# deepspeedai/DeepSpeed

Measured on AMD Instinct MI355X. Metric: tokens/sec Llama-3-8B ZeRO-3, higher is better.
Workload: dtype bf16; 1 GPU; model=llama3-8b, global_batch=8, seq_len=4096, parallelism=zero3_dp1, grad_accum=2

## Files before the change

deepspeed_amd/ops/csrc/attention_bwd.hip:

```cpp
#include <torch/extension.h>

#include "common.h"

using bf16x8_t = __attribute__((ext_vector_type(8))) short;
using f32x4_t = __attribute__((ext_vector_type(4))) float;
using u32x4_t = __attribute__((ext_vector_type(4))) unsigned int;
using u32x2_t = __attribute__((ext_vector_type(2))) unsigned int;

#define MFMA_BF16_16x16x32 __builtin_amdgcn_mfma_f32_16x16x32_bf16

namespace bwd {

constexpr int BR = 128;
constexpr int WR = 32;
constexpr int KTW1 = 1;
constexpr int TS = 32;
constexpr int PT = 64;

DEV_INLINE unsigned int cvtpk2(float lo, float hi) {
  unsigned short a = __builtin_bit_cast(unsigned short, (__bf16)lo);
  unsigned short b = __builtin_bit_cast(unsigned short, (__bf16)hi);
  return (unsigned int)a | ((unsigned int)b << 16);
}

template <int DH>
__launch_bounds__(256)
__global__ void bwd_preprocess(
    const short* __restrict__ q, const short* __restrict__ k,
    const short* __restrict__ dout, const short* __restrict__ out,
    const float* __restrict__ lse,
    short* __restrict__ qT, short* __restrict__ doT, short* __restrict__ kT,
    float* __restrict__ drowP, float* __restrict__ lseP,
    int B, int S, int Sp, int Hq, int Hk) {
  constexpr int PPR = DH / 8;
  __shared__ unsigned int t[PT][DH / 2 + 1];

  const int z = blockIdx.z;
  const int H = (z == 2) ? Hk : Hq;
  const int bh = blockIdx.y;
  if (bh >= B * H) return;
  const int b = bh / H;
  const int h = bh % H;
  const int s0 = blockIdx.x * PT;
  const short* src = (z == 0) ? q : (z == 1) ? dout : k;
  short* dst = (z == 0) ? qT : (z == 1) ? doT : kT;

  for (int i = threadIdx.x; i < PT * PPR; i += 256) {
    const int row = i / PPR;
    const int c = i % PPR;
    const int s = s0 + row;
    const long long off = (((long long)b * S + s) * H + h) * DH + c * 8;
    u32x4_t x = {0u, 0u, 0u, 0u};
    if (s < S) x = *reinterpret_cast<const u32x4_t*>(src + off);
#pragma unroll
    for (int w = 0; w < 4; ++w) t[row][c * 4 + w] = x[w];
    if (z == 1) {
      u32x4_t o = {0u, 0u, 0u, 0u};
      if (s < S) o = *reinterpret_cast<const u32x4_t*>(out + off);
      float acc = 0.f;
#pragma unroll
      for (int w = 0; w < 4; ++w)
        acc += bf2f((short)(x[w] & 0xffff)) * bf2f((short)(o[w] & 0xffff)) +
               bf2f((short)(x[w] >> 16)) * bf2f((short)(o[w] >> 16));
#pragma unroll
      for (int m = PPR / 2; m > 0; m >>= 1) acc += __shfl_xor(acc, m, WAVE);
      if (c == 0) drowP[((long long)b * Hq + h) * Sp + s] = acc;
    } else if (z == 0 && c == 0) {
      float l = 0.f;
      if (s < S) {
        l = lse[((long long)b * Hq + h) * S + s];
        if (l == -INFINITY) l = INFINITY;
      }
      lseP[((long long)b * Hq + h) * Sp + s] = l;
    }
  }
  __syncthreads();
  for (int i = threadIdx.x; i < DH * (PT / 8); i += 256) {
    const int d = i / (PT / 8);
    const int pc = i % (PT / 8);
    const int sh = (d & 1) * 16;
    unsigned int e[8];
#pragma unroll
    for (int j = 0; j < 8; ++j) e[j] = (t[pc * 8 + j][d >> 1] >> sh) & 0xffffu;
    u32x4_t y = {e[0] | (e[1] << 16), e[2] | (e[3] << 16),
                 e[4] | (e[5] << 16), e[6] | (e[7] << 16)};
    *reinterpret_cast<u32x4_t*>(dst + (((long long)b * H + h) * DH + d) * Sp +
                                s0 + pc * 8) = y;
  }
}

template <int DH>
DEV_INLINE int rmswz(int row, int byte_off) {
  return row * (DH * 2) + (byte_off ^ ((row & 7) << 4));
}

DEV_INLINE void lds_dma16(const short* src, char* lds_wave_base) {
  __builtin_amdgcn_global_load_lds(
      reinterpret_cast<const unsigned int*>(src),
      reinterpret_cast<unsigned int*>(lds_wave_base), 16, 0, 0);
}

template <int DH>
DEV_INLINE void issue_rm(const short* base, long long rs, int r0, int S,
                         char* img, int sseg, int lane) {
  const int linear = sseg * 1024 + lane * 16;
  const int row = linear / (DH * 2);
  const int colbyte = linear % (DH * 2);
  const int src_col = colbyte ^ ((row & 7) << 4);
  const int grow = r0 + row;
  const int srow = grow < S ? grow : S - 1;
  lds_dma16(base + (long long)srow * rs + (src_col >> 1), img + sseg * 1024);
}

template <int DH>
DEV_INLINE void issue_tr(const short* baseT, int Sp, int c0, char* img,
                         int sseg, int lane) {
  const int linear = sseg * 1024 + lane * 16;
  const int d = linear >> 6;
  const int g = ((linear >> 4) & 3) ^ ((d >> 2) & 3);
  lds_dma16(baseT + (long long)d * Sp + c0 + g * 8, img + sseg * 1024);
}

template <int DH>
DEV_INLINE bf16x8_t read_rm(const char* img, int row, int ks, int l4) {
  return *reinterpret_cast<const bf16x8_t*>(
      img + rmswz<DH>(row, (l4 * 8 + 32 * ks) * 2));
}

DEV_INLINE bf16x8_t read_tr(const char* img, int d, int l4) {
  const int sw = (d >> 2) & 3;
  const char* rowp = img + d * 64 + (l4 & 1) * 8;
  u32x2_t lo = *reinterpret_cast<const u32x2_t*>(rowp + (((l4 >> 1) ^ sw) << 4));
  u32x2_t hi =
      *reinterpret_cast<const u32x2_t*>(rowp + (((2 + (l4 >> 1)) ^ sw) << 4));
  u32x4_t w = {lo[0], lo[1], hi[0], hi[1]};
  return __builtin_bit_cast(bf16x8_t, w);
}

DEV_INLINE bf16x8_t pack_pair(const f32x4_t& a, const f32x4_t& b) {
  u32x4_t w = {cvtpk2(a[0], a[1]), cvtpk2(a[2], a[3]), cvtpk2(b[0], b[1]),
               cvtpk2(b[2], b[3])};
  return __builtin_bit_cast(bf16x8_t, w);
}

DEV_INLINE void store4(short* p, const f32x4_t& a) {
  u32x2_t w = {cvtpk2(a[0], a[1]), cvtpk2(a[2], a[3])};
  *reinterpret_cast<u32x2_t*>(p) = w;
}

template <int NDT, int STRIDE>
DEV_INLINE void unrotate_row(f32x4_t* acc ,
                             const float* __restrict__ cr,
                             const float* __restrict__ sr) {
#pragma unroll
  for (int dt = 0; dt < NDT / 2; ++dt) {
    const f32x4_t c = *reinterpret_cast<const f32x4_t*>(cr + 16 * dt);
    const f32x4_t sn = *reinterpret_cast<const f32x4_t*>(sr + 16 * dt);
    const f32x4_t d1 = acc[dt * STRIDE];
    const f32x4_t d2 = acc[(dt + NDT / 2) * STRIDE];
    acc[dt * STRIDE] = d1 * c + d2 * sn;
    acc[(dt + NDT / 2) * STRIDE] = d2 * c - d1 * sn;
  }
}

template <int DH, int KTW, bool ROPE>
__launch_bounds__(512 / KTW, 1)
__global__ void flash_bwd_dkv_kernel(
    const short* __restrict__ q,
    const short* __restrict__ k,
    const short* __restrict__ v,
    const short* __restrict__ dout,
    const short* __restrict__ qT,
    const short* __restrict__ doT,
    const float* __restrict__ lseP,
    const float* __restrict__ drowP,
    const float* __restrict__ kvmask,
    short* __restrict__ dk,
    short* __restrict__ dv,
    const float* __restrict__ rope_cos,
    const float* __restrict__ rope_sin,
    int B, int S, int Sp, int Hq, int Hk, float scale, int causal) {
  constexpr int NKS = DH / 32;
  constexpr int NDT = DH / 16;
  constexpr int IMG = TS * DH * 2;
  constexpr int SPI = DH / 16;
  constexpr int NW = 8 / KTW;
  constexpr int WRK = 16 * KTW;
  constexpr int LD_OFF = 4 * IMG;
  constexpr int BUF = LD_OFF + 256;
  __shared__ __attribute__((aligned(16))) char smem[2 * BUF];

  const int lane = threadIdx.x & 63;
  const int wave = threadIdx.x >> 6;
  const int l15 = lane & 15;
  const int l4 = lane >> 4;

  const int bh = blockIdx.y;
  const int b = bh / Hk;
  const int hk = bh % Hk;
  const int G = Hq / Hk;
  const int kv_base = blockIdx.x * BR;
  const int wk = kv_base + wave * WRK;

  const long long qrs = (long long)Hq * DH;
  const long long kvrs = (long long)Hk * DH;
  const short* kp = k + ((long long)b * S) * kvrs + hk * DH;
  const short* vp = v + ((long long)b * S) * kvrs + hk * DH;

  bf16x8_t kfrag[KTW][NKS], vfrag[KTW][NKS];
  float maskv[KTW];
#pragma unroll
  for (int kt = 0; kt < KTW; ++kt) {
    const int krow = wk + 16 * kt + l15;
    const int srow = krow < S ? krow : S - 1;
    const short* ks = kp + (long long)srow * kvrs;
    const short* vs = vp + (long long)srow * kvrs;
#pragma unroll
    for (int ks_i = 0; ks_i < NKS; ++ks_i) {
      kfrag[kt][ks_i] =
          *reinterpret_cast<const bf16x8_t*>(ks + ks_i * 32 + l4 * 8);
      vfrag[kt][ks_i] =
          *reinterpret_cast<const bf16x8_t*>(vs + ks_i * 32 + l4 * 8);
    }
    maskv[kt] = (kvmask && krow < S) ? kvmask[(long long)b * S + krow] : 0.f;
  }

  f32x4_t dk_acc[NDT][KTW], dv_acc[NDT][KTW];
#pragma unroll
  for (int dt = 0; dt < NDT; ++dt)
#pragma unroll
    for (int kt = 0; kt < KTW; ++kt) {
      dk_acc[dt][kt] = f32x4_t{0.f, 0.f, 0.f, 0.f};
      dv_acc[dt][kt] = f32x4_t{0.f, 0.f, 0.f, 0.f};
    }

  const int q_start = causal ? kv_base : 0;
  const int nq = (S - q_start + TS - 1) / TS;
  const int total = G * nq;

  auto issue = [&](int g, int qb, int bufi) {
    const int h = hk * G + g;
    char* buf = smem + bufi * BUF;
    const short* qp = q + ((long long)b * S) * qrs + h * DH;
    const short* dop = dout + ((long long)b * S) * qrs + h * DH;
    const long long toff = ((long long)b * Hq + h) * DH * Sp;
    const long long roff = ((long long)b * Hq + h) * Sp;
#pragma unroll
    for (int sseg = wave; sseg < SPI; sseg += NW) {
      issue_rm<DH>(qp, qrs, qb, S, buf, sseg, lane);
      issue_rm<DH>(dop, qrs, qb, S, buf + IMG, sseg, lane);
      issue_tr<DH>(qT + toff, Sp, qb, buf + 2 * IMG, sseg, lane);
      issue_tr<DH>(doT + toff, Sp, qb, buf + 3 * IMG, sseg, lane);
    }
    if (wave == 0) {
      const float* s = (lane < 32 ? lseP : drowP) + roff + qb + (lane & 31);
      __builtin_amdgcn_global_load_lds(
          reinterpret_cast<const unsigned int*>(s),
          reinterpret_cast<unsigned int*>(buf + LD_OFF), 4, 0, 0);
    }
  };

  int g_nx = 0, qb_nx = q_start;
  issue(g_nx, qb_nx, 0);
  for (int it = 0; it < total; ++it) {
    const int qb = qb_nx;
    asm volatile("s_waitcnt vmcnt(0)" ::: "memory");
    __syncthreads();
    qb_nx += TS;
    if (qb_nx >= S) {
      qb_nx = q_start;
      ++g_nx;
    }
    if (it + 1 < total) issue(g_nx, qb_nx, (it + 1) & 1);

    if (wk >= S || (causal && qb + TS - 1 < wk)) continue;
    const bool interior = !kvmask && qb + TS <= S && wk + WRK <= S &&
                          (!causal || qb >= wk + WRK - 1);
    const char* buf = smem + (it & 1) * BUF;
    const float* ld = reinterpret_cast<const float*>(buf + LD_OFF);

    f32x4_t s_acc[2][KTW], dp_acc[2][KTW], lrow[2];
#pragma unroll
    for (int qt = 0; qt < 2; ++qt) {
      lrow[qt] = *reinterpret_cast<const f32x4_t*>(ld + 16 * qt + 4 * l4);
      f32x4_t dr = *reinterpret_cast<const f32x4_t*>(ld + 32 + 16 * qt + 4 * l4);
#pragma unroll
      for (int kt = 0; kt < KTW; ++kt) {
        s_acc[qt][kt] = f32x4_t{0.f, 0.f, 0.f, 0.f};
        dp_acc[qt][kt] = -dr;
      }
    }
    __builtin_amdgcn_s_setprio(1);
#pragma unroll
    for (int qt = 0; qt < 2; ++qt)
#pragma unroll
      for (int ks_i = 0; ks_i < NKS; ++ks_i) {
        bf16x8_t aq = read_rm<DH>(buf, l15 + 16 * qt, ks_i, l4);
        bf16x8_t ad = read_rm<DH>(buf + IMG, l15 + 16 * qt, ks_i, l4);
#pragma unroll
        for (int kt = 0; kt < KTW; ++kt) {
          s_acc[qt][kt] = MFMA_BF16_16x16x32(aq, kfrag[kt][ks_i],
                                             s_acc[qt][kt], 0, 0, 0);
          dp_acc[qt][kt] = MFMA_BF16_16x16x32(ad, vfrag[kt][ks_i],
                                              dp_acc[qt][kt], 0, 0, 0);
        }
      }
    __builtin_amdgcn_s_setprio(0);

    if (interior) {
#pragma unroll
      for (int qt = 0; qt < 2; ++qt)
#pragma unroll
        for (int kt = 0; kt < KTW; ++kt)
#pragma unroll
          for (int r = 0; r < 4; ++r) {
            float p = __expf(s_acc[qt][kt][r] * scale - lrow[qt][r]);
            s_acc[qt][kt][r] = p;
            dp_acc[qt][kt][r] = p * dp_acc[qt][kt][r] * scale;
          }
    } else {
#pragma unroll
      for (int qt = 0; qt < 2; ++qt)
#pragma unroll
        for (int kt = 0; kt < KTW; ++kt) {
          const int gkv = wk + 16 * kt + l15;
#pragma unroll
          for (int r = 0; r < 4; ++r) {
            const int gq = qb + 16 * qt + 4 * l4 + r;
            const bool valid = gq < S && gkv < S && (!causal || gq >= gkv);
            float sval = s_acc[qt][kt][r] * scale + maskv[kt];
            float p = valid ? __expf(sval - lrow[qt][r]) : 0.f;
            s_acc[qt][kt][r] = p;
            dp_acc[qt][kt][r] = p * dp_acc[qt][kt][r] * scale;
          }
        }
    }
    bf16x8_t pb[KTW], dsb[KTW];
#pragma unroll
    for (int kt = 0; kt < KTW; ++kt) {
      pb[kt] = pack_pair(s_acc[0][kt], s_acc[1][kt]);
      dsb[kt] = pack_pair(dp_acc[0][kt], dp_acc[1][kt]);
    }

    __builtin_amdgcn_s_setprio(1);
#pragma unroll
    for (int dt = 0; dt < NDT; ++dt) {
      bf16x8_t aqt = read_tr(buf + 2 * IMG, l15 + 16 * dt, l4);
      bf16x8_t adt = read_tr(buf + 3 * IMG, l15 + 16 * dt, l4);
#pragma unroll
      for (int kt = 0; kt < KTW; ++kt) {
        dv_acc[dt][kt] =
            MFMA_BF16_16x16x32(adt, pb[kt], dv_acc[dt][kt], 0, 0, 0);
        dk_acc[dt][kt] =
            MFMA_BF16_16x16x32(aqt, dsb[kt], dk_acc[dt][kt], 0, 0, 0);
      }
    }
    __builtin_amdgcn_s_setprio(0);
  }

#pragma unroll
  for (int kt = 0; kt < KTW; ++kt) {
    const int gkv = wk + 16 * kt + l15;
    if (gkv >= S) continue;
    short* dkr = dk + ((long long)b * S + gkv) * kvrs + hk * DH + 4 * l4;
    short* dvr = dv + ((long long)b * S + gkv) * kvrs + hk * DH + 4 * l4;
    if (ROPE)
      unrotate_row<NDT, KTW>(&dk_acc[0][kt],
                             rope_cos + (long long)gkv * (DH / 2) + 4 * l4,
                             rope_sin + (long long)gkv * (DH / 2) + 4 * l4);
#pragma unroll
    for (int dt = 0; dt < NDT; ++dt) {
      store4(dkr + 16 * dt, dk_acc[dt][kt]);
      store4(dvr + 16 * dt, dv_acc[dt][kt]);
    }
  }
}

template <int DH, bool ROPE>
__launch_bounds__(256, 2)
__global__ void flash_bwd_dq_kernel(
    const short* __restrict__ q, const short* __restrict__ k,
    const short* __restrict__ v, const short* __restrict__ dout,
    const short* __restrict__ kT,
    const float* __restrict__ lseP,
    const float* __restrict__ drowP,
    const float* __restrict__ kvmask,
    short* __restrict__ dq,
    const float* __restrict__ rope_cos,
    const float* __restrict__ rope_sin,
    int B, int S, int Sp, int Hq, int Hk, float scale, int causal) {
  constexpr int NKS = DH / 32;
  constexpr int NDT = DH / 16;
  constexpr int IMG = TS * DH * 2;
  constexpr int SPI = DH / 16;
  constexpr int IPI = SPI / 4;
  constexpr int BUF = 3 * IMG;
  __shared__ __attribute__((aligned(16))) char smem[2 * BUF];

  const int lane = threadIdx.x & 63;
  const int wave = threadIdx.x >> 6;
  const int l15 = lane & 15;
  const int l4 = lane >> 4;

  const int qtile = gridDim.x - 1 - blockIdx.x;
  const int bh = blockIdx.y;
  const int b = bh / Hq;
  const int h = bh % Hq;
  const int hk = h / (Hq / Hk);
  const int qbase = qtile * BR;
  const int wq = qbase + wave * WR;

  const long long qrs = (long long)Hq * DH;
  const long long kvrs = (long long)Hk * DH;
  const short* qp = q + ((long long)b * S) * qrs + h * DH;
  const short* dop = dout + ((long long)b * S) * qrs + h * DH;
  const short* kp = k + ((long long)b * S) * kvrs + hk * DH;
  const short* vp = v + ((long long)b * S) * kvrs + hk * DH;
  const short* ktp = kT + ((long long)b * Hk + hk) * DH * Sp;
  const float* mp = kvmask ? kvmask + (long long)b * S : nullptr;

  bf16x8_t qfrag[2][NKS], dofrag[2][NKS];
  float lse_l[2], dr_l[2];
#pragma unroll
  for (int qt = 0; qt < 2; ++qt) {
    const int qrow = wq + 16 * qt + l15;
    const int srow = qrow < S ? qrow : S - 1;
    const short* qs = qp + (long long)srow * qrs;
    const short* ds = dop + (long long)srow * qrs;
#pragma unroll
    for (int ks_i = 0; ks_i < NKS; ++ks_i) {
      qfrag[qt][ks_i] =
          *reinterpret_cast<const bf16x8_t*>(qs + ks_i * 32 + l4 * 8);
      dofrag[qt][ks_i] =
          *reinterpret_cast<const bf16x8_t*>(ds + ks_i * 32 + l4 * 8);
    }
    lse_l[qt] = lseP[((long long)b * Hq + h) * Sp + qrow];
    dr_l[qt] = drowP[((long long)b * Hq + h) * Sp + qrow];
  }

  f32x4_t dq_acc[NDT][2];
#pragma unroll
  for (int dt = 0; dt < NDT; ++dt)
#pragma unroll
    for (int qt = 0; qt < 2; ++qt) dq_acc[dt][qt] = f32x4_t{0.f, 0.f, 0.f, 0.f};

  const int kv_end = causal ? min(S, qbase + BR) : S;
  const int n_tiles = (kv_end + TS - 1) / TS;

  auto issue = [&](int kvb, int bufi) {
    char* buf = smem + bufi * BUF;
#pragma unroll
    for (int i = 0; i < IPI; ++i) {
      const int sseg = i * 4 + wave;
      issue_rm<DH>(kp, kvrs, kvb, S, buf, sseg, lane);
      issue_rm<DH>(vp, kvrs, kvb, S, buf + IMG, sseg, lane);
      issue_tr<DH>(ktp, Sp, kvb, buf + 2 * IMG, sseg, lane);
    }
  };

  issue(0, 0);
  for (int t = 0; t < n_tiles; ++t) {
    const int kvb = t * TS;
    asm volatile("s_waitcnt vmcnt(0)" ::: "memory");
    __syncthreads();
    if (t + 1 < n_tiles) issue(kvb + TS, (t + 1) & 1);

    if (wq >= S || (causal && kvb > wq + WR - 1)) continue;
    const bool interior = !mp && kvb + TS <= S && wq + WR <= S &&
                          (!causal || kvb + TS - 1 <= wq);
    const char* buf = smem + (t & 1) * BUF;

    f32x4_t s_acc[2][2], dp_acc[2][2];
#pragma unroll
    for (int kt = 0; kt < 2; ++kt)
#pragma unroll
      for (int qt = 0; qt < 2; ++qt) {
        s_acc[kt][qt] = f32x4_t{0.f, 0.f, 0.f, 0.f};
        dp_acc[kt][qt] =
            f32x4_t{-dr_l[qt], -dr_l[qt], -dr_l[qt], -dr_l[qt]};
      }
    __builtin_amdgcn_s_setprio(1);
#pragma unroll
    for (int kt = 0; kt < 2; ++kt)
#pragma unroll
      for (int ks_i = 0; ks_i < NKS; ++ks_i) {
        bf16x8_t ak = read_rm<DH>(buf, l15 + 16 * kt, ks_i, l4);
        bf16x8_t av = read_rm<DH>(buf + IMG, l15 + 16 * kt, ks_i, l4);
#pragma unroll
        for (int qt = 0; qt < 2; ++qt) {
          s_acc[kt][qt] = MFMA_BF16_16x16x32(ak, qfrag[qt][ks_i],
                                             s_acc[kt][qt], 0, 0, 0);
          dp_acc[kt][qt] = MFMA_BF16_16x16x32(av, dofrag[qt][ks_i],
                                              dp_acc[kt][qt], 0, 0, 0);
        }
      }
    __builtin_amdgcn_s_setprio(0);

    if (interior) {
#pragma unroll
      for (int kt = 0; kt < 2; ++kt)
#pragma unroll
        for (int qt = 0; qt < 2; ++qt)
#pragma unroll
          for (int r = 0; r < 4; ++r) {
            float p = __expf(s_acc[kt][qt][r] * scale - lse_l[qt]);
            dp_acc[kt][qt][r] = p * dp_acc[kt][qt][r] * scale;
          }
    } else {
#pragma unroll
      for (int kt = 0; kt < 2; ++kt)
#pragma unroll
        for (int r = 0; r < 4; ++r) {
          const int gkv = kvb + 16 * kt + 4 * l4 + r;
          const float mv = (mp && gkv < S) ? mp[gkv] : 0.f;
#pragma unroll
          for (int qt = 0; qt < 2; ++qt) {
            const int gq = wq + 16 * qt + l15;
            const bool valid = gq < S && gkv < S && (!causal || gkv <= gq);
            float sval = s_acc[kt][qt][r] * scale + mv;
            float p = valid ? __expf(sval - lse_l[qt]) : 0.f;
            dp_acc[kt][qt][r] = p * dp_acc[kt][qt][r] * scale;
          }
        }
    }
    bf16x8_t dsb[2];
#pragma unroll
    for (int qt = 0; qt < 2; ++qt)
      dsb[qt] = pack_pair(dp_acc[0][qt], dp_acc[1][qt]);

    __builtin_amdgcn_s_setprio(1);
#pragma unroll
    for (int dt = 0; dt < NDT; ++dt) {
      bf16x8_t akt = read_tr(buf + 2 * IMG, l15 + 16 * dt, l4);
#pragma unroll
      for (int qt = 0; qt < 2; ++qt)
        dq_acc[dt][qt] =
            MFMA_BF16_16x16x32(akt, dsb[qt], dq_acc[dt][qt], 0, 0, 0);
    }
    __builtin_amdgcn_s_setprio(0);
  }

#pragma unroll
  for (int qt = 0; qt < 2; ++qt) {
    const int gq = wq + 16 * qt + l15;
    if (gq >= S) continue;
    short* dqr = dq + ((long long)b * S + gq) * qrs + h * DH + 4 * l4;
    if (ROPE)
      unrotate_row<NDT, 2>(&dq_acc[0][qt],
                           rope_cos + (long long)gq * (DH / 2) + 4 * l4,
                           rope_sin + (long long)gq * (DH / 2) + 4 * l4);
#pragma unroll
    for (int dt = 0; dt < NDT; ++dt) store4(dqr + 16 * dt, dq_acc[dt][qt]);
  }
}

}

template <int DH, bool ROPE>
static void launch_bwd(at::Tensor& q, at::Tensor& k, at::Tensor& v,
                       at::Tensor& dout, at::Tensor& out, at::Tensor& lse,
                       at::Tensor& dq, at::Tensor& dk, at::Tensor& dv,
                       const float* mp, const float* cosp, const float* sinp,
                       int B, int S, int Hq, int Hk, float scale,
                       int causal) {
  auto stream = c10::hip::getCurrentHIPStream();
  const int Sp = (S + bwd::BR - 1) / bwd::BR * bwd::BR;
  auto qT = at::empty({B, Hq, DH, Sp}, q.options());
  auto doT = at::empty({B, Hq, DH, Sp}, q.options());
  auto kT = at::empty({B, Hk, DH, Sp}, q.options());
  auto drow = at::empty({B, Hq, Sp}, q.options().dtype(at::kFloat));
  auto lseP = at::empty({B, Hq, Sp}, q.options().dtype(at::kFloat));
  auto sp = [](const at::Tensor& t) {
    return reinterpret_cast<const short*>(t.data_ptr());
  };
  auto spm = [](at::Tensor& t) {
    return reinterpret_cast<short*>(t.data_ptr());
  };
  dim3 grid0(Sp / bwd::PT, B * Hq, 3);
  hipLaunchKernelGGL(bwd::bwd_preprocess<DH>, grid0, dim3(256), 0,
                     stream.stream(), sp(q), sp(k), sp(dout), sp(out),
                     lse.data_ptr<float>(), spm(qT), spm(doT), spm(kT),
                     drow.data_ptr<float>(), lseP.data_ptr<float>(), B, S,
                     Sp, Hq, Hk);
  HIP_CHECK_KERNEL();
  dim3 grid1(Sp / bwd::BR, B * Hk);
  hipLaunchKernelGGL((bwd::flash_bwd_dkv_kernel<DH, bwd::KTW1, ROPE>), grid1,
                     dim3(512 / bwd::KTW1), 0, stream.stream(), sp(q), sp(k),
                     sp(v), sp(dout), sp(qT), sp(doT), lseP.data_ptr<float>(),
                     drow.data_ptr<float>(), mp, spm(dk), spm(dv), cosp, sinp,
                     B, S, Sp, Hq, Hk, scale, causal);
  HIP_CHECK_KERNEL();
  dim3 grid2(Sp / bwd::BR, B * Hq);
  hipLaunchKernelGGL((bwd::flash_bwd_dq_kernel<DH, ROPE>), grid2, dim3(256), 0,
                     stream.stream(), sp(q), sp(k), sp(v), sp(dout), sp(kT),
                     lseP.data_ptr<float>(), drow.data_ptr<float>(), mp,
                     spm(dq), cosp, sinp, B, S, Sp, Hq, Hk, scale, causal);
  HIP_CHECK_KERNEL();
}

void flash_check_qkv(const at::Tensor& q, const at::Tensor& k,
                     const at::Tensor& v, const char* who);
const float* flash_check_kvmask(const c10::optional<at::Tensor>& kvmask,
                                const at::Tensor& q);
void check_rope_table(const at::Tensor& cos, const at::Tensor& sin,
                      const at::Tensor& ref, long long S, int D,
                      const char* who);

std::vector<at::Tensor> flash_attn_bwd(at::Tensor q, at::Tensor k,
                                       at::Tensor v, at::Tensor dout,
                                       at::Tensor out, at::Tensor lse,
                                       bool causal, double scale,
                                       c10::optional<at::Tensor> kvmask,
                                       c10::optional<at::Tensor> cos,
                                       c10::optional<at::Tensor> sin) {
  flash_check_qkv(q, k, v, "flash_attn_bwd");
  CHECK_ARG(dout, at::kBFloat16);
  CHECK_ARG(out, at::kBFloat16);
  CHECK_ARG(lse, at::kFloat);
  CHECK_ON(dout, q);
  CHECK_ON(out, q);
  CHECK_ON(lse, q);
  TORCH_CHECK(dout.sizes() == q.sizes() && out.sizes() == q.sizes(),
              "flash_attn_bwd: dout and out must have q's shape");
  int B = q.size(0), S = q.size(1), Hq = q.size(2), D = q.size(3);
  int Hk = k.size(2);
  TORCH_CHECK(lse.dim() == 3 && lse.size(0) == B && lse.size(1) == Hq &&
                  lse.size(2) == S,
              "flash_attn_bwd: lse must be [B,Hq,S]");
  const float* mp = flash_check_kvmask(kvmask, q);
  const float fscale =
      scale == 0.0 ? 1.0f / std::sqrt((float)D) : (float)scale;
  auto dq = at::empty_like(q);
  auto dk = at::empty_like(k);
  auto dv = at::empty_like(v);
  TORCH_CHECK(cos.has_value() == sin.has_value(),
              "flash_attn_bwd: cos and sin must be given together");
  const bool rope = cos.has_value();
  const float* cosp = nullptr;
  const float* sinp = nullptr;
  if (rope) {
    check_rope_table(*cos, *sin, q, S, D, "flash_attn_bwd");
    cosp = cos->data_ptr<float>();
    sinp = sin->data_ptr<float>();
  }
  const int ic = causal ? 1 : 0;
#define DSAMD_LAUNCH_BWD(DH_, ROPE_)                                        \
  launch_bwd<DH_, ROPE_>(q, k, v, dout, out, lse, dq, dk, dv, mp, cosp, sinp, \
                         B, S, Hq, Hk, fscale, ic)
  if (D == 128) {
    if (rope) DSAMD_LAUNCH_BWD(128, true); else DSAMD_LAUNCH_BWD(128, false);
  } else {
    if (rope) DSAMD_LAUNCH_BWD(64, true); else DSAMD_LAUNCH_BWD(64, false);
  }
#undef DSAMD_LAUNCH_BWD
  return {dq, dk, dv};
}
```

Measured before the change: 17360 tokens/s.

## Replace pre-transposed Q/dO/K copies with LDS transpose reads in flash backward

The preprocess kernel no longer writes transposed copies of Q, dO and K to global memory. The dkv and dq kernels instead read the transposed operands directly from the row-major LDS images with ds_read_b64_tr_b16, double-buffering these reads against the MFMAs. A new shared layout header defines a swizzle that serves both row and transposed reads. This removes a full extra global write and read of Q, dO and K, plus the extra DMA into LDS, and halves the LDS image footprint. The cost is inline asm with manual lgkmcnt waits and a new swizzle whose bank-conflict behaviour and correctness depend on the transpose-read semantics.

```diff
diff --git a/deepspeed_amd/ops/csrc/attention_bwd.hip b/deepspeed_amd/ops/csrc/attention_bwd.hip
--- a/deepspeed_amd/ops/csrc/attention_bwd.hip
+++ b/deepspeed_amd/ops/csrc/attention_bwd.hip
@@ -1,6 +1,7 @@
 #include <torch/extension.h>
 
 #include "common.h"
+#include "flash_bwd_layout.h"
 
 using bf16x8_t = __attribute__((ext_vector_type(8))) short;
 using f32x4_t = __attribute__((ext_vector_type(4))) float;
@@ -15,6 +16,7 @@
 constexpr int WR = 32;
 constexpr int KTW1 = 1;
 constexpr int TS = 32;
+static_assert(TS == bwd_layout::TS, "the image layout is for 32-row steps");
 constexpr int PT = 64;
 
 DEV_INLINE unsigned int cvtpk2(float lo, float hi) {
@@ -26,72 +28,44 @@
 template <int DH>
 __launch_bounds__(256)
 __global__ void bwd_preprocess(
-    const short* __restrict__ q, const short* __restrict__ k,
     const short* __restrict__ dout, const short* __restrict__ out,
     const float* __restrict__ lse,
-    short* __restrict__ qT, short* __restrict__ doT, short* __restrict__ kT,
     float* __restrict__ drowP, float* __restrict__ lseP,
-    int B, int S, int Sp, int Hq, int Hk) {
+    int B, int S, int Sp, int Hq) {
   constexpr int PPR = DH / 8;
-  __shared__ unsigned int t[PT][DH / 2 + 1];
-
-  const int z = blockIdx.z;
-  const int H = (z == 2) ? Hk : Hq;
   const int bh = blockIdx.y;
-  if (bh >= B * H) return;
-  const int b = bh / H;
-  const int h = bh % H;
+  const int b = bh / Hq;
+  const int h = bh % Hq;
   const int s0 = blockIdx.x * PT;
-  const short* src = (z == 0) ? q : (z == 1) ? dout : k;
-  short* dst = (z == 0) ? qT : (z == 1) ? doT : kT;
 
   for (int i = threadIdx.x; i < PT * PPR; i += 256) {
     const int row = i / PPR;
     const int c = i % PPR;
     const int s = s0 + row;
-    const long long off = (((long long)b * S + s) * H + h) * DH + c * 8;
+    const long long off = (((long long)b * S + s) * Hq + h) * DH + c * 8;
     u32x4_t x = {0u, 0u, 0u, 0u};
-    if (s < S) x = *reinterpret_cast<const u32x4_t*>(src + off);
-#pragma unroll
-    for (int w = 0; w < 4; ++w) t[row][c * 4 + w] = x[w];
-    if (z == 1) {
-      u32x4_t o = {0u, 0u, 0u, 0u};
-      if (s < S) o = *reinterpret_cast<const u32x4_t*>(out + off);
-      float acc = 0.f;
-#pragma unroll
-      for (int w = 0; w < 4; ++w)
-        acc += bf2f((short)(x[w] & 0xffff)) * bf2f((short)(o[w] & 0xffff)) +
-               bf2f((short)(x[w] >> 16)) * bf2f((short)(o[w] >> 16));
-#pragma unroll
-      for (int m = PPR / 2; m > 0; m >>= 1) acc += __shfl_xor(acc, m, WAVE);
-      if (c == 0) drowP[((long long)b * Hq + h) * Sp + s] = acc;
-    } else if (z == 0 && c == 0) {
+    u32x4_t o = {0u, 0u, 0u, 0u};
+    if (s < S) {
+      x = *reinterpret_cast<const u32x4_t*>(dout + off);
+      o = *reinterpret_cast<const u32x4_t*>(out + off);
+    }
+    float acc = 0.f;
+#pragma unroll
+    for (int w = 0; w < 4; ++w)
+      acc += bf2f((short)(x[w] & 0xffff)) * bf2f((short)(o[w] & 0xffff)) +
+             bf2f((short)(x[w] >> 16)) * bf2f((short)(o[w] >> 16));
+#pragma unroll
+    for (int m = PPR / 2; m > 0; m >>= 1) acc += __shfl_xor(acc, m, WAVE);
+    if (c == 0) {
       float l = 0.f;
       if (s < S) {
         l = lse[((long long)b * Hq + h) * S + s];
         if (l == -INFINITY) l = INFINITY;
       }
+      drowP[((long long)b * Hq + h) * Sp + s] = acc;
       lseP[((long long)b * Hq + h) * Sp + s] = l;
     }
   }
-  __syncthreads();
-  for (int i = threadIdx.x; i < DH * (PT / 8); i += 256) {
-    const int d = i / (PT / 8);
-    const int pc = i % (PT / 8);
-    const int sh = (d & 1) * 16;
-    unsigned int e[8];
-#pragma unroll
-    for (int j = 0; j < 8; ++j) e[j] = (t[pc * 8 + j][d >> 1] >> sh) & 0xffffu;
-    u32x4_t y = {e[0] | (e[1] << 16), e[2] | (e[3] << 16),
-                 e[4] | (e[5] << 16), e[6] | (e[7] << 16)};
-    *reinterpret_cast<u32x4_t*>(dst + (((long long)b * H + h) * DH + d) * Sp +
-                                s0 + pc * 8) = y;
-  }
-}
-
-template <int DH>
-DEV_INLINE int rmswz(int row, int byte_off) {
-  return row * (DH * 2) + (byte_off ^ ((row & 7) << 4));
 }
 
 DEV_INLINE void lds_dma16(const short* src, char* lds_wave_base) {
@@ -104,36 +78,51 @@
 DEV_INLINE void issue_rm(const short* base, long long rs, int r0, int S,
                          char* img, int sseg, int lane) {
   const int linear = sseg * 1024 + lane * 16;
-  const int row = linear / (DH * 2);
-  const int colbyte = linear % (DH * 2);
-  const int src_col = colbyte ^ ((row & 7) << 4);
-  const int grow = r0 + row;
+  const int src_col = bwd_layout::dma_src_byte<DH>(linear);
+  const int grow = r0 + bwd_layout::dma_row<DH>(linear);
   const int srow = grow < S ? grow : S - 1;
   lds_dma16(base + (long long)srow * rs + (src_col >> 1), img + sseg * 1024);
-}
-
-template <int DH>
-DEV_INLINE void issue_tr(const short* baseT, int Sp, int c0, char* img,
-                         int sseg, int lane) {
-  const int linear = sseg * 1024 + lane * 16;
-  const int d = linear >> 6;
-  const int g = ((linear >> 4) & 3) ^ ((d >> 2) & 3);
-  lds_dma16(baseT + (long long)d * Sp + c0 + g * 8, img + sseg * 1024);
 }
 
 template <int DH>
 DEV_INLINE bf16x8_t read_rm(const char* img, int row, int ks, int l4) {
   return *reinterpret_cast<const bf16x8_t*>(
-      img + rmswz<DH>(row, (l4 * 8 + 32 * ks) * 2));
-}
-
-DEV_INLINE bf16x8_t read_tr(const char* img, int d, int l4) {
-  const int sw = (d >> 2) & 3;
-  const char* rowp = img + d * 64 + (l4 & 1) * 8;
-  u32x2_t lo = *reinterpret_cast<const u32x2_t*>(rowp + (((l4 >> 1) ^ sw) << 4));
-  u32x2_t hi =
-      *reinterpret_cast<const u32x2_t*>(rowp + (((2 + (l4 >> 1)) ^ sw) << 4));
-  u32x4_t w = {lo[0], lo[1], hi[0], hi[1]};
+      img + bwd_layout::img_off<DH>(row, (l4 * 8 + 32 * ks) * 2));
+}
+
+DEV_INLINE unsigned lds_addr(const char* p) {
+  return (unsigned)(size_t)(
+      (const __attribute__((address_space(3))) char*)p);
+}
+
+struct tr_frag {
+  u32x2_t lo, hi;
+};
+
+template <int DH>
+DEV_INLINE tr_frag issue_tr_read(unsigned img, int dt, int lane) {
+  tr_frag f;
+  const unsigned a0 = img + bwd_layout::tr_read_addr<DH>(lane, dt, 0);
+  const unsigned a1 = img + bwd_layout::tr_read_addr<DH>(lane, dt, 1);
+  asm volatile("ds_read_b64_tr_b16 %0, %1" : "=v"(f.lo) : "v"(a0) : "memory");
+  asm volatile("ds_read_b64_tr_b16 %0, %1" : "=v"(f.hi) : "v"(a1) : "memory");
+  return f;
+}
+
+template <int N>
+DEV_INLINE void tr_wait(tr_frag& a, tr_frag& b) {
+  asm volatile("s_waitcnt lgkmcnt(%4)"
+               : "+v"(a.lo), "+v"(a.hi), "+v"(b.lo), "+v"(b.hi)
+               : "n"(N));
+}
+
+template <int N>
+DEV_INLINE void tr_wait(tr_frag& a) {
+  asm volatile("s_waitcnt lgkmcnt(%2)" : "+v"(a.lo), "+v"(a.hi) : "n"(N));
+}
+
+DEV_INLINE bf16x8_t tr_operand(const tr_frag& f) {
+  u32x4_t w = {f.lo[0], f.lo[1], f.hi[0], f.hi[1]};
   return __builtin_bit_cast(bf16x8_t, w);
 }
 
@@ -170,8 +159,6 @@
     const short* __restrict__ k,
     const short* __restrict__ v,
     const short* __restrict__ dout,
-    const short* __restrict__ qT,
-    const short* __restrict__ doT,
     const float* __restrict__ lseP,
     const float* __restrict__ drowP,
     const float* __restrict__ kvmask,
@@ -186,12 +173,12 @@
   constexpr int SPI = DH / 16;
   constexpr int NW = 8 / KTW;
   constexpr int WRK = 16 * KTW;
-  constexpr int LD_OFF = 4 * IMG;
+  constexpr int LD_OFF = 2 * IMG;
   constexpr int BUF = LD_OFF + 256;
   __shared__ __attribute__((aligned(16))) char smem[2 * BUF];
 
   const int lane = threadIdx.x & 63;
-  const int wave = threadIdx.x >> 6;
+  const int wave = __builtin_amdgcn_readfirstlane(threadIdx.x >> 6);
   const int l15 = lane & 15;
   const int l4 = lane >> 4;
 
@@ -224,6 +211,15 @@
     }
     maskv[kt] = (kvmask && krow < S) ? kvmask[(long long)b * S + krow] : 0.f;
   }
+#pragma unroll
+  for (int kt = 0; kt < KTW; ++kt) {
+#pragma unroll
+    for (int ks_i = 0; ks_i < NKS; ++ks_i) {
+      asm volatile("" : "+v"(kfrag[kt][ks_i]));
+      asm volatile("" : "+v"(vfrag[kt][ks_i]));
+    }
+    asm volatile("" : "+v"(maskv[kt]));
+  }
 
   f32x4_t dk_acc[NDT][KTW], dv_acc[NDT][KTW];
 #pragma unroll
@@ -238,19 +234,16 @@
   const int nq = (S - q_start + TS - 1) / TS;
   const int total = G * nq;
 
+  static_assert(SPI <= NW, "one image segment per wave at the most");
   auto issue = [&](int g, int qb, int bufi) {
     const int h = hk * G + g;
     char* buf = smem + bufi * BUF;
     const short* qp = q + ((long long)b * S) * qrs + h * DH;
     const short* dop = dout + ((long long)b * S) * qrs + h * DH;
-    const long long toff = ((long long)b * Hq + h) * DH * Sp;
     const long long roff = ((long long)b * Hq + h) * Sp;
-#pragma unroll
-    for (int sseg = wave; sseg < SPI; sseg += NW) {
-      issue_rm<DH>(qp, qrs, qb, S, buf, sseg, lane);
-      issue_rm<DH>(dop, qrs, qb, S, buf + IMG, sseg, lane);
-      issue_tr<DH>(qT + toff, Sp, qb, buf + 2 * IMG, sseg, lane);
-      issue_tr<DH>(doT + toff, Sp, qb, buf + 3 * IMG, sseg, lane);
+    if (wave < SPI) {
+      issue_rm<DH>(qp, qrs, qb, S, buf, wave, lane);
+      issue_rm<DH>(dop, qrs, qb, S, buf + IMG, wave, lane);
     }
     if (wave == 0) {
       const float* s = (lane < 32 ? lseP : drowP) + roff + qb + (lane & 31);
@@ -265,7 +258,8 @@
   for (int it = 0; it < total; ++it) {
     const int qb = qb_nx;
     asm volatile("s_waitcnt vmcnt(0)" ::: "memory");
-    __syncthreads();
+    __builtin_amdgcn_s_barrier();
+    asm volatile("" ::: "memory");
     qb_nx += TS;
     if (qb_nx >= S) {
       qb_nx = q_start;
@@ -342,11 +336,22 @@
       dsb[kt] = pack_pair(dp_acc[0][kt], dp_acc[1][kt]);
     }
 
+    const unsigned qimg = lds_addr(buf);
+    tr_frag fq[2], fd[2];
+    fq[0] = issue_tr_read<DH>(qimg, 0, lane);
+    fd[0] = issue_tr_read<DH>(qimg + IMG, 0, lane);
     __builtin_amdgcn_s_setprio(1);
 #pragma unroll
     for (int dt = 0; dt < NDT; ++dt) {
-      bf16x8_t aqt = read_tr(buf + 2 * IMG, l15 + 16 * dt, l4);
-      bf16x8_t adt = read_tr(buf + 3 * IMG, l15 + 16 * dt, l4);
+      if (dt + 1 < NDT) {
+        fq[(dt + 1) & 1] = issue_tr_read<DH>(qimg, dt + 1, lane);
+        fd[(dt + 1) & 1] = issue_tr_read<DH>(qimg + IMG, dt + 1, lane);
+        tr_wait<4>(fq[dt & 1], fd[dt & 1]);
+      } else {
+        tr_wait<0>(fq[dt & 1], fd[dt & 1]);
+      }
+      const bf16x8_t aqt = tr_operand(fq[dt & 1]);
+      const bf16x8_t adt = tr_operand(fd[dt & 1]);
 #pragma unroll
       for (int kt = 0; kt < KTW; ++kt) {
         dv_acc[dt][kt] =
@@ -381,7 +386,6 @@
 __global__ void flash_bwd_dq_kernel(
     const short* __restrict__ q, const short* __restrict__ k,
     const short* __restrict__ v, const short* __restrict__ dout,
-    const short* __restrict__ kT,
     const float* __restrict__ lseP,
     const float* __restrict__ drowP,
     const float* __restrict__ kvmask,
@@ -394,7 +398,7 @@
   constexpr int IMG = TS * DH * 2;
   constexpr int SPI = DH / 16;
   constexpr int IPI = SPI / 4;
-  constexpr int BUF = 3 * IMG;
+  constexpr int BUF = 2 * IMG;
   __shared__ __attribute__((aligned(16))) char smem[2 * BUF];
 
   const int lane = threadIdx.x & 63;
@@ -416,7 +420,6 @@
   const short* dop = dout + ((long long)b * S) * qrs + h * DH;
   const short* kp = k + ((long long)b * S) * kvrs + hk * DH;
   const short* vp = v + ((long long)b * S) * kvrs + hk * DH;
-  const short* ktp = kT + ((long long)b * Hk + hk) * DH * Sp;
   const float* mp = kvmask ? kvmask + (long long)b * S : nullptr;
 
   bf16x8_t qfrag[2][NKS], dofrag[2][NKS];
@@ -454,7 +457,6 @@
       const int sseg = i * 4 + wave;
       issue_rm<DH>(kp, kvrs, kvb, S, buf, sseg, lane);
       issue_rm<DH>(vp, kvrs, kvb, S, buf + IMG, sseg, lane);
-      issue_tr<DH>(ktp, Sp, kvb, buf + 2 * IMG, sseg, lane);
     }
   };
 
@@ -528,10 +530,19 @@
     for (int qt = 0; qt < 2; ++qt)
       dsb[qt] = pack_pair(dp_acc[0][qt], dp_acc[1][qt]);
 
+    const unsigned kimg = lds_addr(buf);
+    tr_frag fk[2];
+    fk[0] = issue_tr_read<DH>(kimg, 0, lane);
     __builtin_amdgcn_s_setprio(1);
 #pragma unroll
     for (int dt = 0; dt < NDT; ++dt) {
-      bf16x8_t akt = read_tr(buf + 2 * IMG, l15 + 16 * dt, l4);
+      if (dt + 1 < NDT) {
+        fk[(dt + 1) & 1] = issue_tr_read<DH>(kimg, dt + 1, lane);
+        tr_wait<2>(fk[dt & 1]);
+      } else {
+        tr_wait<0>(fk[dt & 1]);
+      }
+      const bf16x8_t akt = tr_operand(fk[dt & 1]);
 #pragma unroll
       for (int qt = 0; qt < 2; ++qt)
         dq_acc[dt][qt] =
@@ -565,9 +576,6 @@
                        int causal) {
   auto stream = c10::hip::getCurrentHIPStream();
   const int Sp = (S + bwd::BR - 1) / bwd::BR * bwd::BR;
-  auto qT = at::empty({B, Hq, DH, Sp}, q.options());
-  auto doT = at::empty({B, Hq, DH, Sp}, q.options());
-  auto kT = at::empty({B, Hk, DH, Sp}, q.options());
   auto drow = at::empty({B, Hq, Sp}, q.options().dtype(at::kFloat));
   auto lseP = at::empty({B, Hq, Sp}, q.options().dtype(at::kFloat));
   auto sp = [](const at::Tensor& t) {
@@ -576,23 +584,22 @@
   auto spm = [](at::Tensor& t) {
     return reinterpret_cast<short*>(t.data_ptr());
   };
-  dim3 grid0(Sp / bwd::PT, B * Hq, 3);
+  dim3 grid0(Sp / bwd::PT, B * Hq);
   hipLaunchKernelGGL(bwd::bwd_preprocess<DH>, grid0, dim3(256), 0,
-                     stream.stream(), sp(q), sp(k), sp(dout), sp(out),
-                     lse.data_ptr<float>(), spm(qT), spm(doT), spm(kT),
-                     drow.data_ptr<float>(), lseP.data_ptr<float>(), B, S,
-                     Sp, Hq, Hk);
+                     stream.stream(), sp(dout), sp(out),
+                     lse.data_ptr<float>(), drow.data_ptr<float>(),
+                     lseP.data_ptr<float>(), B, S, Sp, Hq);
   HIP_CHECK_KERNEL();
   dim3 grid1(Sp / bwd::BR, B * Hk);
   hipLaunchKernelGGL((bwd::flash_bwd_dkv_kernel<DH, bwd::KTW1, ROPE>), grid1,
                      dim3(512 / bwd::KTW1), 0, stream.stream(), sp(q), sp(k),
-                     sp(v), sp(dout), sp(qT), sp(doT), lseP.data_ptr<float>(),
+                     sp(v), sp(dout), lseP.data_ptr<float>(),
                      drow.data_ptr<float>(), mp, spm(dk), spm(dv), cosp, sinp,
                      B, S, Sp, Hq, Hk, scale, causal);
   HIP_CHECK_KERNEL();
   dim3 grid2(Sp / bwd::BR, B * Hq);
   hipLaunchKernelGGL((bwd::flash_bwd_dq_kernel<DH, ROPE>), grid2, dim3(256), 0,
-                     stream.stream(), sp(q), sp(k), sp(v), sp(dout), sp(kT),
+                     stream.stream(), sp(q), sp(k), sp(v), sp(dout),
                      lseP.data_ptr<float>(), drow.data_ptr<float>(), mp,
                      spm(dq), cosp, sinp, B, S, Sp, Hq, Hk, scale, causal);
   HIP_CHECK_KERNEL();
diff --git a/deepspeed_amd/ops/csrc/flash_bwd_layout.h b/deepspeed_amd/ops/csrc/flash_bwd_layout.h
--- /dev/null
+++ b/deepspeed_amd/ops/csrc/flash_bwd_layout.h
@@ -0,0 +1,48 @@
+#pragma once
+
+#if defined(__HIPCC__)
+#define FBL_HD __host__ __device__ __forceinline__
+#else
+#define FBL_HD inline
+#endif
+
+namespace bwd_layout {
+
+constexpr int TS = 32;
+
+template <int DH>
+FBL_HD int img_xor(int row) {
+  constexpr int RB = DH * 2;
+  constexpr int RPB = 256 / RB;
+  constexpr int NP = RB / 32;
+  return ((row / RPB) & (NP - 1)) << 5;
+}
+
+template <int DH>
+FBL_HD int img_off(int row, int byte_off) {
+  return row * (DH * 2) + (byte_off ^ img_xor<DH>(row));
+}
+
+template <int DH>
+FBL_HD int dma_row(int linear) {
+  return linear / (DH * 2);
+}
+template <int DH>
+FBL_HD int dma_src_byte(int linear) {
+  return (linear % (DH * 2)) ^ img_xor<DH>(dma_row<DH>(linear));
+}
+
+template <int DH>
+FBL_HD int row_read_addr(int lane, int rt, int ks) {
+  const int l15 = lane & 15, l4 = lane >> 4;
+  return img_off<DH>(16 * rt + l15, (32 * ks + 8 * l4) * 2);
+}
+
+template <int DH>
+FBL_HD int tr_read_addr(int lane, int dt, int hf) {
+  const int l15 = lane & 15, l4 = lane >> 4;
+  const int q = l15 >> 2, p = l15 & 3;
+  return img_off<DH>(16 * hf + 4 * l4 + q, 32 * dt + 8 * p);
+}
+
+}
```

Measured after the change: 18350 tokens/s (median of 6 runs). +5.7%, better.
